# kaixi287/rsl_rl

Measured on AMD Instinct MI355X. Metric: PPO env-steps/sec (rollout+GAE+update) at N=65536 envs, 1→8 MI355X, higher is better.
Workload: dtype fp32

## Files before the change

rsl_rl_amd/csrc/mlp_fwd_stream.hip:

```cpp
#include <cstring>

#include "common.h"
#include "fwd_stream.h"
#include "mlp_tile.h"
#include "ppo_loss_common.h"
#include "x6_split.h"

namespace rslrl {
namespace {

constexpr int kFsT = 128;
constexpr int kFsN = 256;
constexpr int kFsThreads = 512;
constexpr int kFsChunkB = kFsT * 32;
constexpr int kFsMaxSlices = 128;
constexpr int kFsImgPlaneU = kX6PlaneB / 16;
constexpr int kFsImgChunkU = kX6ChunkB / 16;
static_assert(kFsT == kBM && kFsN == kBN && kFsThreads == kThreads, "the tiled kernel's tile (mlp_tile.h)");
constexpr uint32_t kFsRsrcFlags = 0x00020000;
#ifndef RSLRL_FS_LA
#define RSLRL_FS_LA 1
#endif
constexpr bool kFsLA = RSLRL_FS_LA != 0;

template <int K>
struct FsCfg {
    static constexpr int kChunks = K / 16;
    static constexpr int kStages = K == 256 ? 4 : 1;
    static constexpr int kNch = kChunks / kStages;
    static constexpr int kCols = 16 * kNch;
    static constexpr int kPlaneB = kNch * kFsChunkB;
    static constexpr int kBufB = 3 * kPlaneB;
    static constexpr int kUnitsRow = kCols / 4;
    static constexpr int kUpt = kFsT * kUnitsRow / kFsThreads;
    static_assert(K == 256 || K == 48, "streaming forward: K = 256 or 48");
    static_assert(kNch >= 2 && kUpt <= 4 && kFsT * kUnitsRow % kFsThreads == 0, "stage shape");
};

struct FsProblem {
    const float* x;
    const uint4* img;
    const float* bias;
    float* h;
};

struct FsArgs {
    FsProblem p[2];
    int tiles;
    int tiles_per;
};

__host__ __device__ constexpr int fs_f(int c) { return (c & 3) | ((c & 1) << 2); }

__device__ __forceinline__ int fs_off(int m, int col) {
    const int c = col >> 4;
    return c * kFsChunkB + (m ^ fs_f(c)) * 32 + 16 * (((col >> 3) & 1) ^ ((m >> 3) & 1)) + 8 * ((col >> 2) & 1);
}

__device__ __forceinline__ bf16x8 fs_read16(int addr) {
    typedef __attribute__((address_space(3))) uint4 lds_u4;
    return __builtin_bit_cast(bf16x8, *reinterpret_cast<const lds_u4*>(addr));
}

template <int K>
__device__ __forceinline__ void fs_load_x(__amdgpu_buffer_rsrc_t r, int q, float4 (&v)[4]) {
    using C = FsCfg<K>;
#pragma unroll
    for (int j = 0; j < C::kUpt; ++j) {
        const int u = threadIdx.x + kFsThreads * j;
        const int off = ((u / C::kUnitsRow) * K + 4 * (u % C::kUnitsRow)) * 4;
        v[j] = __builtin_bit_cast(float4, __builtin_amdgcn_raw_buffer_load_b128(r, off, q * C::kCols * 4, 2));
    }
}

template <int K>
__device__ __forceinline__ void fs_store_x1(const float4& v, int j, char* __restrict__ buf) {
    using C = FsCfg<K>;
    uint2 w[3];
    split4(v, w[0], w[1], w[2]);
    const int u = threadIdx.x + kFsThreads * j;
    const int off = fs_off(u / C::kUnitsRow, 4 * (u % C::kUnitsRow));
#pragma unroll
    for (int q = 0; q < 3; ++q) *reinterpret_cast<uint2*>(buf + q * C::kPlaneB + off) = w[q];
}

template <int K>
__global__ __launch_bounds__(kFsThreads, 1) void fwd_stream_kernel(FsArgs args) {
    using C = FsCfg<K>;
    __shared__ __attribute__((aligned(16))) char lds[2 * C::kBufB];
    const FsProblem& P = args.p[blockIdx.y];
    const int t_begin = blockIdx.x * args.tiles_per;
    const int t_end = min(args.tiles, t_begin + args.tiles_per);
    if (t_begin >= t_end) return;

    const int lane = threadIdx.x & 63;
    const int wave = __builtin_amdgcn_readfirstlane(threadIdx.x >> 6);
    if (wave >= 4) __builtin_amdgcn_s_setprio(1);
    const int h = lane >> 5;
    const int l32 = lane & 31;

    const int lbase = static_cast<int>(reinterpret_cast<uintptr_t>(lds));
    int la[2][C::kNch];
#pragma unroll
    for (int c = 0; c < C::kNch; ++c) {
        la[0][c] = lbase + fs_off(l32, 16 * c + 8 * h);
        la[1][c] = la[0][c] + C::kBufB;
    }
    const int brow = 32 * wave + l32;
    const int boff = (brow * 2 + (h ^ ((brow >> 3) & 1))) * 16;
    const __amdgpu_buffer_rsrc_t rimg = __builtin_amdgcn_make_buffer_rsrc(
        const_cast<uint4*>(P.img), 0, static_cast<uint32_t>(C::kChunks * kFsImgChunkU * 16), kFsRsrcFlags);
    auto bload = [&](int c, int q) {
        return __builtin_bit_cast(uint4, __builtin_amdgcn_raw_buffer_load_b128(rimg, boff, (c * kFsImgChunkU + q * kFsImgPlaneU) * 16, 0));
    };
    const float bias = P.bias[32 * wave + l32];

    auto tile_rsrc = [&](int tile) {
        return __builtin_amdgcn_make_buffer_rsrc(const_cast<float*>(P.x + static_cast<int64_t>(tile) * kFsT * K), 0,
                                                 static_cast<uint32_t>(kFsT * K * 4), kFsRsrcFlags);
    };

    float4 xr[4];
    fs_load_x<K>(tile_rsrc(t_begin), 0, xr);
#pragma unroll
    for (int j = 0; j < C::kUpt; ++j) fs_store_x1<K>(xr[j], j, lds);
    if (C::kStages > 1) fs_load_x<K>(tile_rsrc(t_begin), 1, xr);
    else if (t_begin + 1 < t_end) fs_load_x<K>(tile_rsrc(t_begin + 1), 0, xr);
    __syncthreads();

    uint4 bq[2][3];
#pragma unroll
    for (int q = 0; q < 3; ++q) bq[0][q] = bload(0, q);

    auto epi_part = [&](const f32x16 (&acc)[4], int tile, int e) {
        const __amdgpu_buffer_rsrc_t rc = __builtin_amdgcn_make_buffer_rsrc(
            P.h + static_cast<int64_t>(tile) * kFsT * kFsN + 32 * wave, 0, static_cast<uint32_t>(kFsT * kFsN * 4),
            kFsRsrcFlags);
        const int i = e >> 2;
#pragma unroll
        for (int k = 0; k < 4; ++k) {
            const int r = 4 * (e & 3) + k;
            float v = acc[i][r] + bias;
            const float n = elu_neg(fminf(v, 0.f));
            v = v > 0.f ? v : n;
            __builtin_amdgcn_raw_buffer_store_b32(__builtin_bit_cast(uint32_t, v), rc, ((4 * h + (r & 3)) * kFsN + l32) * 4,
                                                  (32 * i + 8 * (r >> 2)) * kFsN * 4, 2 );
        }
    };

    auto run_tile = [&](int tile, f32x16 (&acc)[4], const f32x16 (&prev)[4], bool has_prev, int par) {
        const bool more = tile + 1 < t_end;
#pragma unroll
        for (int kq = 0; kq < C::kStages; ++kq) {
            const int buf = (C::kStages % 2 == 0) ? (kq & 1) : (par ^ (kq & 1));
            bf16x8 an[3];
            if constexpr (kFsLA) {
                an[0] = fs_read16(la[buf][0]);
                an[1] = fs_read16(la[buf][0] + C::kPlaneB);
                an[2] = fs_read16(la[buf][0] + 2 * C::kPlaneB);
            }
            const bool next_stage = kq + 1 < C::kStages || more;
#pragma unroll
            for (int c = 0; c < C::kNch; ++c) {
                const int gc = C::kNch * kq + c;
                const int slot = (par * C::kChunks + gc) & 1;
#pragma unroll
                for (int q = 0; q < 3; ++q) bq[slot ^ 1][q] = bload((gc + 1) % C::kChunks, q);
                bf16x8 bf[3];
#pragma unroll
                for (int q = 0; q < 3; ++q) bf[q] = __builtin_bit_cast(bf16x8, bq[slot][q]);
#pragma unroll
                for (int i = 0; i < 4; ++i) {
                    const int blk = 4 * c + i;
                    bf16x8 af[3];
                    if constexpr (kFsLA) {
#pragma unroll
                        for (int q = 0; q < 3; ++q) af[q] = an[q];
                        if (blk + 1 < 4 * C::kNch) {
                            const int a1 = la[buf][(blk + 1) >> 2] + ((blk + 1) & 3) * 1024;
                            an[0] = fs_read16(a1);
                            an[1] = fs_read16(a1 + C::kPlaneB);
                            an[2] = fs_read16(a1 + 2 * C::kPlaneB);
                        }
                    } else {
                        const int a0 = la[buf][c] + i * 1024;
                        af[0] = fs_read16(a0);
                        af[1] = fs_read16(a0 + C::kPlaneB);
                        af[2] = fs_read16(a0 + 2 * C::kPlaneB);
                    }
                    acc[i] = mfma_x6(af, bf, gc == 0 ? f32x16{} : acc[i]);
                    if (kq == 0 && has_prev) {
                        if (blk < 16) epi_part(prev, tile - 1, blk);
                        if (blk == 4 * C::kNch - 1) {
#pragma unroll
                            for (int e = 4 * C::kNch; e < 16; ++e) epi_part(prev, tile - 1, e);
                        }
                    }
                    if (c == 1 && i < C::kUpt && next_stage) fs_store_x1<K>(xr[i], i, lds + (buf ^ 1) * C::kBufB);
                    __builtin_amdgcn_sched_barrier(0);
                }
                if (c == C::kNch - 1) {
                    if (C::kStages > 1) {
                        if (kq < C::kStages - 2 || more) {
                            const int s2 = kq + 2;
                            fs_load_x<K>(tile_rsrc(s2 < C::kStages ? tile : tile + 1), s2 % C::kStages, xr);
                        }
                    } else if (tile + 2 < t_end) {
                        fs_load_x<K>(tile_rsrc(tile + 2), 0, xr);
                    }
                    __builtin_amdgcn_sched_barrier(0);
                }
            }
            __syncthreads();
        }
    };

    f32x16 acc0[4], acc1[4];
    int tile = t_begin;
    for (; tile + 1 < t_end; tile += 2) {
        run_tile(tile, acc0, acc1, tile > t_begin, 0);
        run_tile(tile + 1, acc1, acc0, true, 1);
    }
    if (tile < t_end) {
        run_tile(tile, acc0, acc1, tile > t_begin, 0);
#pragma unroll
        for (int e = 0; e < 16; ++e) epi_part(acc0, tile, e);
    } else {
#pragma unroll
        for (int e = 0; e < 16; ++e) epi_part(acc1, tile - 1, e);
    }
}


struct VhArgs {
    const float* x;
    const uint4* img;
    const float* bias;
    const float* wv;
    float bv;
    const float* bvp;
    const float* tv;
    const float* ret;
    float* dz;
    float* y;
    float* wpart;
    float clip, g;
    int clipped;
    int tiles, tiles_per;
};
constexpr int kVhP = 260;

__global__ __launch_bounds__(kFsThreads, 1) void value_head_stream_kernel(VhArgs a) {
    using C = FsCfg<256>;
    __shared__ __attribute__((aligned(16))) char lds[2 * C::kBufB];
    __shared__ float red[8 * kFsT];
    __shared__ float dvl[kFsT];
    __shared__ float dbred[kFsT / 64];
    const int t_begin = blockIdx.x * a.tiles_per;
    const int t_end = min(a.tiles, t_begin + a.tiles_per);
    if (t_begin >= t_end) return;

    const int lane = threadIdx.x & 63;
    const int wave = __builtin_amdgcn_readfirstlane(threadIdx.x >> 6);
    if (wave >= 4) __builtin_amdgcn_s_setprio(1);
    const int h = lane >> 5;
    const int l32 = lane & 31;

    const int lbase = static_cast<int>(reinterpret_cast<uintptr_t>(lds));
    int la[2][C::kNch];
#pragma unroll
    for (int c = 0; c < C::kNch; ++c) {
        la[0][c] = lbase + fs_off(l32, 16 * c + 8 * h);
        la[1][c] = la[0][c] + C::kBufB;
    }
    const int brow = 32 * wave + l32;
    const int boff = (brow * 2 + (h ^ ((brow >> 3) & 1))) * 16;
    const __amdgpu_buffer_rsrc_t rimg = __builtin_amdgcn_make_buffer_rsrc(
        const_cast<uint4*>(a.img), 0, static_cast<uint32_t>(C::kChunks * kFsImgChunkU * 16), kFsRsrcFlags);
    auto bload = [&](int c, int q) {
        return __builtin_bit_cast(uint4, __builtin_amdgcn_raw_buffer_load_b128(rimg, boff, (c * kFsImgChunkU + q * kFsImgPlaneU) * 16, 0));
    };
    float bcol[16], wcol[16];
#pragma unroll
    for (int g = 0; g < 4; ++g) {
        const float4 b4 = *reinterpret_cast<const float4*>(a.bias + 32 * wave + 8 * g + 4 * h);
        const float4 w4 = *reinterpret_cast<const float4*>(a.wv + 32 * wave + 8 * g + 4 * h);
        bcol[4 * g] = b4.x; bcol[4 * g + 1] = b4.y; bcol[4 * g + 2] = b4.z; bcol[4 * g + 3] = b4.w;
        wcol[4 * g] = w4.x; wcol[4 * g + 1] = w4.y; wcol[4 * g + 2] = w4.z; wcol[4 * g + 3] = w4.w;
    }
    const float bv = *a.bvp;
    auto tile_rsrc = [&](int tile) {
        return __builtin_amdgcn_make_buffer_rsrc(const_cast<float*>(a.x + static_cast<int64_t>(tile) * kFsT * 256), 0,
                                                 static_cast<uint32_t>(kFsT * 256 * 4), kFsRsrcFlags);
    };

    float4 xr[4];
    fs_load_x<256>(tile_rsrc(t_begin), 0, xr);
#pragma unroll
    for (int j = 0; j < C::kUpt; ++j) fs_store_x1<256>(xr[j], j, lds);
    fs_load_x<256>(tile_rsrc(t_begin), 1, xr);
    __syncthreads();

    uint4 bq[2][3];
#pragma unroll
    for (int q = 0; q < 3; ++q) bq[0][q] = bload(0, q);

    float wacc[16];
#pragma unroll
    for (int r = 0; r < 16; ++r) wacc[r] = 0.f;
    float dbacc = 0.f;

    for (int tile = t_begin; tile < t_end; ++tile) {
        const bool more = tile + 1 < t_end;
        const int64_t row0 = static_cast<int64_t>(tile) * kFsT;
        f32x16 acc[4];
#pragma unroll
        for (int kq = 0; kq < 4; ++kq) {
            const int buf = kq & 1;
            bf16x8 an[3];
            an[0] = fs_read16(la[buf][0]);
            an[1] = fs_read16(la[buf][0] + C::kPlaneB);
            an[2] = fs_read16(la[buf][0] + 2 * C::kPlaneB);
#pragma unroll
            for (int c = 0; c < C::kNch; ++c) {
                const int gc = C::kNch * kq + c;
                const int slot = gc & 1;
#pragma unroll
                for (int q = 0; q < 3; ++q) bq[slot ^ 1][q] = bload((gc + 1) % C::kChunks, q);
                bf16x8 bf[3];
#pragma unroll
                for (int q = 0; q < 3; ++q) bf[q] = __builtin_bit_cast(bf16x8, bq[slot][q]);
#pragma unroll
                for (int i = 0; i < 4; ++i) {
                    const int blk = 4 * c + i;
                    bf16x8 af[3];
#pragma unroll
                    for (int q = 0; q < 3; ++q) af[q] = an[q];
                    if (blk + 1 < 4 * C::kNch) {
                        const int a1 = la[buf][(blk + 1) >> 2] + ((blk + 1) & 3) * 1024;
                        an[0] = fs_read16(a1);
                        an[1] = fs_read16(a1 + C::kPlaneB);
                        an[2] = fs_read16(a1 + 2 * C::kPlaneB);
                    }
                    acc[i] = mfma_x6(bf, af, gc == 0 ? f32x16{} : acc[i]);
                    if (c == 1 && i < C::kUpt && (kq < 3 || more)) fs_store_x1<256>(xr[i], i, lds + (buf ^ 1) * C::kBufB);
                    __builtin_amdgcn_sched_barrier(0);
                }
                if (c == C::kNch - 1) {
                    if (kq < 2 || more) fs_load_x<256>(tile_rsrc(kq < 2 ? tile : tile + 1), (kq + 2) & 3, xr);
                    __builtin_amdgcn_sched_barrier(0);
                }
            }
            __syncthreads();
        }
        float tvr = 0.f, retr = 0.f;
        if (threadIdx.x < kFsT) {
            tvr = a.tv[row0 + threadIdx.x];
            retr = a.ret[row0 + threadIdx.x];
        }
#pragma unroll
        for (int i = 0; i < 4; ++i) {
            float oval = 0.f;
#pragma unroll
            for (int r = 0; r < 16; ++r) {
                const float tt = acc[i][r] + bcol[r];
                const float n = elu_neg(fminf(tt, 0.f));
                const float hv = tt > 0.f ? tt : n;
                acc[i][r] = hv;
                oval = fmaf(hv, wcol[r], oval);
            }
            const float tsum = oval + __shfl_xor(oval, 32, 64);
            if (h == 0) red[wave * kFsT + 32 * i + l32] = tsum;
        }
        __syncthreads();
        if (threadIdx.x < kFsT) {
            const int rl = threadIdx.x;
            float V = red[rl];
#pragma unroll
            for (int w = 1; w < 8; ++w) V += red[w * kFsT + rl];
            V += bv;
            a.y[row0 + rl] = V;
            const float dV = value_loss_grad(V, tvr, retr, a.clipped, a.clip, a.g);
            dvl[rl] = dV;
            dbacc += dV;
        }
        __syncthreads();
        float* dzt = a.dz + row0 * 256 + 32 * wave + 4 * h;
#pragma unroll
        for (int i = 0; i < 4; ++i) {
            const float dv = dvl[32 * i + l32];
#pragma unroll
            for (int g = 0; g < 4; ++g) {
                float o[4];
#pragma unroll
                for (int k = 0; k < 4; ++k) {
                    const int r = 4 * g + k;
                    const float hh = acc[i][r];
                    const float z = __fmaf_rn(dv, wcol[r], 0.f);
                    o[k] = hh > 0.f ? z : z * (hh + 1.f);
                    wacc[r] = fmaf(dv, hh, wacc[r]);
                }
                const f32x4 ov = {o[0], o[1], o[2], o[3]};
                *reinterpret_cast<f32x4*>(dzt + (32 * i + l32) * 256 + 8 * g) = ov;
            }
        }
    }
    float* wp = a.wpart + static_cast<int64_t>(blockIdx.x) * kVhP;
#pragma unroll
    for (int r = 0; r < 16; ++r) {
        float v = wacc[r];
#pragma unroll
        for (int off = 1; off < 32; off <<= 1) v += __shfl_xor(v, off, 64);
        wacc[r] = v;
    }
    if (l32 == 0) {
#pragma unroll
        for (int g = 0; g < 4; ++g)
            *reinterpret_cast<float4*>(wp + 32 * wave + 8 * g + 4 * h) =
                make_float4(wacc[4 * g], wacc[4 * g + 1], wacc[4 * g + 2], wacc[4 * g + 3]);
    }
    if (threadIdx.x < kFsT) {
        float v = dbacc;
#pragma unroll
        for (int off = 1; off < 64; off <<= 1) v += __shfl_xor(v, off, 64);
        if (lane == 0) dbred[wave] = v;
    }
    __syncthreads();
    if (threadIdx.x == 0) {
        wp[256] = dbred[0] + dbred[1];
        wp[257] = 0.f;
        wp[258] = 0.f;
        wp[259] = 0.f;
    }
}

int64_t fs_tiles_per(int64_t tiles) { return ceil_div(tiles, std::min<int64_t>(kFsMaxSlices, tiles)); }

}

bool fwd_stream_forced() {
    static const bool on = [] {
        const char* e = std::getenv("RSLRL_FWD_STREAM");
        return e && (std::strcmp(e, "1") == 0 || std::strcmp(e, "48") == 0);
    }();
    return on;
}

bool fwd_stream48() {
    static const bool on = [] {
        const char* e = std::getenv("RSLRL_FWD_STREAM");
        return e && std::strcmp(e, "48") == 0;
    }();
    return on;
}

bool fwd_stream_enabled() {
    static const bool on = [] {
        const char* e = std::getenv("RSLRL_FWD_STREAM");
        return !(e && e[0] == '0');
    }();
    return on;
}

int fwd_stream_pair(const FwdStreamProblem* p, int n, int64_t M, int K, hipStream_t st) {
    if (n < 1 || n > 2 || M <= 0 || M % kFsT || M / kFsT > INT32_MAX || (K != 256 && K != 48))
        return RSLRL_E_UNSUPPORTED;
    FsArgs args{};
    for (int i = 0; i < n; ++i) {
        const uintptr_t bits = reinterpret_cast<uintptr_t>(p[i].x) | reinterpret_cast<uintptr_t>(p[i].img);
        if (!p[i].x || !p[i].img || !p[i].bias || !p[i].h) return RSLRL_E_INVALID_ARGUMENT;
        if (bits & 15) return RSLRL_E_MISALIGNED;
        args.p[i] = FsProblem{p[i].x, static_cast<const uint4*>(p[i].img), p[i].bias, p[i].h};
    }
    const int64_t tiles = M / kFsT;
    const int64_t per = fs_tiles_per(tiles);
    args.tiles = static_cast<int>(tiles);
    args.tiles_per = static_cast<int>(per);
    const dim3 grid(static_cast<unsigned>(ceil_div(tiles, per)), static_cast<unsigned>(n));
    if (K == 256) hipLaunchKernelGGL(fwd_stream_kernel<256>, grid, dim3(kFsThreads), 0, st, args);
    else hipLaunchKernelGGL(fwd_stream_kernel<48>, grid, dim3(kFsThreads), 0, st, args);
    return launch_status();
}


int value_head_stream(const ValueHeadStreamArgs& v, hipStream_t st) {
    if (v.M <= 0 || v.M % kFsT || v.M / kFsT > INT32_MAX) return RSLRL_E_UNSUPPORTED;
    const uintptr_t bits = reinterpret_cast<uintptr_t>(v.x) | reinterpret_cast<uintptr_t>(v.img) |
                           reinterpret_cast<uintptr_t>(v.bias) | reinterpret_cast<uintptr_t>(v.wv) |
                           reinterpret_cast<uintptr_t>(v.dz) | reinterpret_cast<uintptr_t>(v.wpart);
    if (bits & 15) return RSLRL_E_MISALIGNED;
    const int64_t tiles = v.M / kFsT;
    const int64_t per = ceil_div(tiles, std::min<int64_t>(2 * kFsMaxSlices, tiles));
    VhArgs a{};
    a.x = v.x;
    a.img = static_cast<const uint4*>(v.img);
    a.bias = v.bias;
    a.wv = v.wv;
    a.bvp = v.bv;
    a.tv = v.tv;
    a.ret = v.ret;
    a.dz = v.dz;
    a.y = v.y;
    a.wpart = v.wpart;
    a.clip = v.clip;
    a.g = v.g;
    a.clipped = v.clipped;
    a.tiles = static_cast<int>(tiles);
    a.tiles_per = static_cast<int>(per);
    hipLaunchKernelGGL(value_head_stream_kernel, dim3(static_cast<unsigned>(ceil_div(tiles, per))), dim3(kFsThreads), 0,
                       st, a);
    return launch_status();
}

int64_t value_head_stream_rows(int64_t M) {
    if (M <= 0 || M % kFsT) return 0;
    const int64_t tiles = M / kFsT;
    const int64_t per = ceil_div(tiles, std::min<int64_t>(2 * kFsMaxSlices, tiles));
    return ceil_div(tiles, per);
}

bool value_head_stream_enabled() {
    static const bool on = [] {
        const char* e = std::getenv("RSLRL_VALUE_HEAD_STREAM");
        return !(e && e[0] == '0');
    }();
    return on;
}
}
```

Measured before the change: 18.87 million.

## Overlap value-head epilogue of previous tile with next tile's MFMA main loop

Result: no change. 18.94 million, median of 6 (+0.4%).

```diff
diff --git a/rsl_rl_amd/csrc/mlp_fwd_stream.hip b/rsl_rl_amd/csrc/mlp_fwd_stream.hip
--- a/rsl_rl_amd/csrc/mlp_fwd_stream.hip
+++ b/rsl_rl_amd/csrc/mlp_fwd_stream.hip
@@ -249,13 +249,17 @@
     int tiles, tiles_per;
 };
 constexpr int kVhP = 260;
-
+constexpr bool kVhOverlapDefault = true;
+
+template <bool kOverlap>
 __global__ __launch_bounds__(kFsThreads, 1) void value_head_stream_kernel(VhArgs a) {
     using C = FsCfg<256>;
     __shared__ __attribute__((aligned(16))) char lds[2 * C::kBufB];
     __shared__ float red[8 * kFsT];
     __shared__ float dvl[kFsT];
     __shared__ float dbred[kFsT / 64];
+    __shared__ __attribute__((aligned(16))) float btab[kOverlap ? kFsN : 4];
+    __shared__ __attribute__((aligned(16))) float wtab[kOverlap ? kFsN : 4];
     const int t_begin = blockIdx.x * a.tiles_per;
     const int t_end = min(a.tiles, t_begin + a.tiles_per);
     if (t_begin >= t_end) return;
@@ -281,24 +285,57 @@
         return __builtin_bit_cast(uint4, __builtin_amdgcn_raw_buffer_load_b128(rimg, boff, (c * kFsImgChunkU + q * kFsImgPlaneU) * 16, 0));
     };
     float bcol[16], wcol[16];
-#pragma unroll
-    for (int g = 0; g < 4; ++g) {
-        const float4 b4 = *reinterpret_cast<const float4*>(a.bias + 32 * wave + 8 * g + 4 * h);
-        const float4 w4 = *reinterpret_cast<const float4*>(a.wv + 32 * wave + 8 * g + 4 * h);
-        bcol[4 * g] = b4.x; bcol[4 * g + 1] = b4.y; bcol[4 * g + 2] = b4.z; bcol[4 * g + 3] = b4.w;
-        wcol[4 * g] = w4.x; wcol[4 * g + 1] = w4.y; wcol[4 * g + 2] = w4.z; wcol[4 * g + 3] = w4.w;
-    }
+    if constexpr (kOverlap) {
+        if (threadIdx.x < kFsN) {
+            btab[threadIdx.x] = a.bias[threadIdx.x];
+            wtab[threadIdx.x] = a.wv[threadIdx.x];
+        }
+    } else {
+#pragma unroll
+        for (int g = 0; g < 4; ++g) {
+            const float4 b4 = *reinterpret_cast<const float4*>(a.bias + 32 * wave + 8 * g + 4 * h);
+            const float4 w4 = *reinterpret_cast<const float4*>(a.wv + 32 * wave + 8 * g + 4 * h);
+            bcol[4 * g] = b4.x; bcol[4 * g + 1] = b4.y; bcol[4 * g + 2] = b4.z; bcol[4 * g + 3] = b4.w;
+            wcol[4 * g] = w4.x; wcol[4 * g + 1] = w4.y; wcol[4 * g + 2] = w4.z; wcol[4 * g + 3] = w4.w;
+        }
+    }
+    auto col4 = [&](const float (&reg)[16], const float* tab, int g, float (&o)[4]) {
+        if constexpr (kOverlap) {
+            int off = 4 * h;
+            asm volatile("" : "+v"(off));
+            const float4 v = *reinterpret_cast<const float4*>(tab + 32 * wave + 8 * g + off);
+            o[0] = v.x; o[1] = v.y; o[2] = v.z; o[3] = v.w;
+        } else {
+#pragma unroll
+            for (int k = 0; k < 4; ++k) o[k] = reg[4 * g + k];
+        }
+    };
     const float bv = *a.bvp;
     auto tile_rsrc = [&](int tile) {
         return __builtin_amdgcn_make_buffer_rsrc(const_cast<float*>(a.x + static_cast<int64_t>(tile) * kFsT * 256), 0,
                                                  static_cast<uint32_t>(kFsT * 256 * 4), kFsRsrcFlags);
     };
 
+    const int xg = ((threadIdx.x / C::kUnitsRow) * 256 + 4 * (threadIdx.x % C::kUnitsRow)) * 4;
+    const int xl = fs_off(threadIdx.x / C::kUnitsRow, 4 * (threadIdx.x % C::kUnitsRow));
+    static_assert(kFsThreads / C::kUnitsRow == 32 && C::kUpt == 4, "unit j = unit 0 + 32 j rows");
     float4 xr[4];
-    fs_load_x<256>(tile_rsrc(t_begin), 0, xr);
-#pragma unroll
-    for (int j = 0; j < C::kUpt; ++j) fs_store_x1<256>(xr[j], j, lds);
-    fs_load_x<256>(tile_rsrc(t_begin), 1, xr);
+    auto load_x = [&](__amdgpu_buffer_rsrc_t r, int q) {
+#pragma unroll
+        for (int j = 0; j < 4; ++j)
+            xr[j] = __builtin_bit_cast(float4, __builtin_amdgcn_raw_buffer_load_b128(r, xg, q * C::kCols * 4 + j * 32 * 256 * 4, 2));
+    };
+    auto store_x1 = [&](int j, int buf) {
+        uint2 w[3];
+        split4(xr[j], w[0], w[1], w[2]);
+#pragma unroll
+        for (int q = 0; q < 3; ++q)
+            *reinterpret_cast<uint2*>(lds + xl + (buf * C::kBufB + q * C::kPlaneB + j * 1024)) = w[q];
+    };
+    load_x(tile_rsrc(t_begin), 0);
+#pragma unroll
+    for (int j = 0; j < 4; ++j) store_x1(j, 0);
+    load_x(tile_rsrc(t_begin), 1);
     __syncthreads();
 
     uint4 bq[2][3];
@@ -309,18 +346,103 @@
 #pragma unroll
     for (int r = 0; r < 16; ++r) wacc[r] = 0.f;
     float dbacc = 0.f;
-
-    for (int tile = t_begin; tile < t_end; ++tile) {
+    float tvr = 0.f, retr = 0.f;
+    float oval = 0.f;
+    float dvc = 0.f;
+
+    auto row_rsrc = [&](const float* p, int tile) {
+        return __builtin_amdgcn_make_buffer_rsrc(const_cast<float*>(p + static_cast<int64_t>(tile) * kFsT), 0,
+                                                 static_cast<uint32_t>(kFsT * 4), kFsRsrcFlags);
+    };
+    auto load_targets = [&](int tile) {
+        if (wave < kFsT / 64) {
+            tvr = __builtin_bit_cast(float, __builtin_amdgcn_raw_buffer_load_b32(row_rsrc(a.tv, tile), 4 * threadIdx.x, 0, 0));
+            retr = __builtin_bit_cast(float, __builtin_amdgcn_raw_buffer_load_b32(row_rsrc(a.ret, tile), 4 * threadIdx.x, 0, 0));
+        }
+    };
+    auto stage_a = [&](f32x16 (&acc)[4], int i, int g) {
+        float b4[4], w4[4];
+        col4(bcol, btab, g, b4);
+        col4(wcol, wtab, g, w4);
+        if (g == 0) oval = 0.f;
+#pragma unroll
+        for (int k = 0; k < 4; ++k) {
+            const int r = 4 * g + k;
+            const float tt = acc[i][r] + b4[k];
+            const float n = elu_neg(fminf(tt, 0.f));
+            const float hv = tt > 0.f ? tt : n;
+            acc[i][r] = hv;
+            oval = fmaf(hv, w4[k], oval);
+        }
+        if (g == 3) {
+            const float tsum = oval + __shfl_xor(oval, 32, 64);
+            if (h == 0) red[wave * kFsT + 32 * i + l32] = tsum;
+        }
+    };
+    auto stage_b = [&](int tile) {
+        if (wave < kFsT / 64) {
+            const int rl = threadIdx.x;
+            float V = red[rl];
+#pragma unroll
+            for (int w = 1; w < 8; ++w) V += red[w * kFsT + rl];
+            V += bv;
+            __builtin_amdgcn_raw_buffer_store_b32(__builtin_bit_cast(uint32_t, V), row_rsrc(a.y, tile), 4 * rl, 0, 0);
+            const float dV = value_loss_grad(V, tvr, retr, a.clipped, a.clip, a.g);
+            dvl[rl] = dV;
+            dbacc += dV;
+        }
+    };
+    auto stage_c = [&](const f32x16 (&acc)[4], int tile, int i, int g) {
+        const uint64_t dzb = reinterpret_cast<uint64_t>(a.dz + static_cast<int64_t>(tile) * kFsT * 256 + 32 * wave + 32 * i * 256 + 8 * g);
+        const uint32_t dzlo = __builtin_amdgcn_readfirstlane(static_cast<uint32_t>(dzb));
+        const uint32_t dzhi = __builtin_amdgcn_readfirstlane(static_cast<uint32_t>(dzb >> 32));
+        typedef __attribute__((address_space(1))) f32x4 global_f32x4;
+        if (g == 0) dvc = dvl[32 * i + l32];
+        float w4[4];
+        col4(wcol, wtab, g, w4);
+        float o[4];
+#pragma unroll
+        for (int k = 0; k < 4; ++k) {
+            const int r = 4 * g + k;
+            const float hh = acc[i][r];
+            const float z = __fmaf_rn(dvc, w4[k], 0.f);
+            o[k] = hh > 0.f ? z : z * (hh + 1.f);
+            wacc[r] = fmaf(dvc, hh, wacc[r]);
+        }
+        const f32x4 ov = {o[0], o[1], o[2], o[3]};
+        *reinterpret_cast<global_f32x4*>((static_cast<uint64_t>(dzhi) << 32 | dzlo) +
+                                         static_cast<uint32_t>((l32 * 256 + 4 * h) * 4)) = ov;
+    };
+    auto drain = [&](f32x16 (&acc)[4], int tile) {
+        load_targets(tile);
+#pragma unroll
+        for (int i = 0; i < 4; ++i) {
+#pragma unroll
+            for (int g = 0; g < 4; ++g) stage_a(acc, i, g);
+        }
+        __syncthreads();
+        stage_b(tile);
+        __syncthreads();
+#pragma unroll
+        for (int i = 0; i < 4; ++i) {
+#pragma unroll
+            for (int g = 0; g < 4; ++g) stage_c(acc, tile, i, g);
+        }
+    };
+
+    auto run_tile = [&](int tile, f32x16 (&acc)[4], f32x16 (&prev)[4], bool has_prev) {
         const bool more = tile + 1 < t_end;
-        const int64_t row0 = static_cast<int64_t>(tile) * kFsT;
-        f32x16 acc[4];
+        const bool epi = kOverlap && has_prev;
 #pragma unroll
         for (int kq = 0; kq < 4; ++kq) {
             const int buf = kq & 1;
+            const bool look = !(kOverlap && kq == 0);
             bf16x8 an[3];
-            an[0] = fs_read16(la[buf][0]);
-            an[1] = fs_read16(la[buf][0] + C::kPlaneB);
-            an[2] = fs_read16(la[buf][0] + 2 * C::kPlaneB);
+            if (look) {
+                an[0] = fs_read16(la[buf][0]);
+                an[1] = fs_read16(la[buf][0] + C::kPlaneB);
+                an[2] = fs_read16(la[buf][0] + 2 * C::kPlaneB);
+            }
 #pragma unroll
             for (int c = 0; c < C::kNch; ++c) {
                 const int gc = C::kNch * kq + c;
@@ -334,75 +456,62 @@
                 for (int i = 0; i < 4; ++i) {
                     const int blk = 4 * c + i;
                     bf16x8 af[3];
-#pragma unroll
-                    for (int q = 0; q < 3; ++q) af[q] = an[q];
-                    if (blk + 1 < 4 * C::kNch) {
-                        const int a1 = la[buf][(blk + 1) >> 2] + ((blk + 1) & 3) * 1024;
-                        an[0] = fs_read16(a1);
-                        an[1] = fs_read16(a1 + C::kPlaneB);
-                        an[2] = fs_read16(a1 + 2 * C::kPlaneB);
+                    if (look) {
+#pragma unroll
+                        for (int q = 0; q < 3; ++q) af[q] = an[q];
+                        if (blk + 1 < 4 * C::kNch) {
+                            const int a1 = la[buf][(blk + 1) >> 2] + ((blk + 1) & 3) * 1024;
+                            an[0] = fs_read16(a1);
+                            an[1] = fs_read16(a1 + C::kPlaneB);
+                            an[2] = fs_read16(a1 + 2 * C::kPlaneB);
+                        }
+                    } else {
+                        const int a0 = la[buf][c] + i * 1024;
+                        af[0] = fs_read16(a0);
+                        af[1] = fs_read16(a0 + C::kPlaneB);
+                        af[2] = fs_read16(a0 + 2 * C::kPlaneB);
                     }
                     acc[i] = mfma_x6(bf, af, gc == 0 ? f32x16{} : acc[i]);
-                    if (c == 1 && i < C::kUpt && (kq < 3 || more)) fs_store_x1<256>(xr[i], i, lds + (buf ^ 1) * C::kBufB);
+                    if constexpr (kOverlap) {
+                        if (epi) {
+                            if (kq == 0) stage_a(prev, blk >> 2, blk & 3);
+                            if (kq == 1 && blk == 0) stage_b(tile - 1);
+                            if (kq == 2) stage_c(prev, tile - 1, blk >> 2, blk & 3);
+                        }
+                    }
+                    if (c == 1 && (kq < 3 || more)) store_x1(i, buf ^ 1);
                     __builtin_amdgcn_sched_barrier(0);
                 }
                 if (c == C::kNch - 1) {
-                    if (kq < 2 || more) fs_load_x<256>(tile_rsrc(kq < 2 ? tile : tile + 1), (kq + 2) & 3, xr);
+                    if (kq < 2 || more) load_x(tile_rsrc(kq < 2 ? tile : tile + 1), (kq + 2) & 3);
+                    if constexpr (kOverlap) {
+                        if (kq == 0 && epi) load_targets(tile - 1);
+                    }
                     __builtin_amdgcn_sched_barrier(0);
                 }
             }
             __syncthreads();
         }
-        float tvr = 0.f, retr = 0.f;
-        if (threadIdx.x < kFsT) {
-            tvr = a.tv[row0 + threadIdx.x];
-            retr = a.ret[row0 + threadIdx.x];
-        }
-#pragma unroll
-        for (int i = 0; i < 4; ++i) {
-            float oval = 0.f;
-#pragma unroll
-            for (int r = 0; r < 16; ++r) {
-                const float tt = acc[i][r] + bcol[r];
-                const float n = elu_neg(fminf(tt, 0.f));
-                const float hv = tt > 0.f ? tt : n;
-                acc[i][r] = hv;
-                oval = fmaf(hv, wcol[r], oval);
-            }
-            const float tsum = oval + __shfl_xor(oval, 32, 64);
-            if (h == 0) red[wave * kFsT + 32 * i + l32] = tsum;
-        }
-        __syncthreads();
-        if (threadIdx.x < kFsT) {
-            const int rl = threadIdx.x;
-            float V = red[rl];
-#pragma unroll
-            for (int w = 1; w < 8; ++w) V += red[w * kFsT + rl];
-            V += bv;
-            a.y[row0 + rl] = V;
-            const float dV = value_loss_grad(V, tvr, retr, a.clipped, a.clip, a.g);
-            dvl[rl] = dV;
-            dbacc += dV;
-        }
-        __syncthreads();
-        float* dzt = a.dz + row0 * 256 + 32 * wave + 4 * h;
-#pragma unroll
-        for (int i = 0; i < 4; ++i) {
-            const float dv = dvl[32 * i + l32];
-#pragma unroll
-            for (int g = 0; g < 4; ++g) {
-                float o[4];
-#pragma unroll
-                for (int k = 0; k < 4; ++k) {
-                    const int r = 4 * g + k;
-                    const float hh = acc[i][r];
-                    const float z = __fmaf_rn(dv, wcol[r], 0.f);
-                    o[k] = hh > 0.f ? z : z * (hh + 1.f);
-                    wacc[r] = fmaf(dv, hh, wacc[r]);
-                }
-                const f32x4 ov = {o[0], o[1], o[2], o[3]};
-                *reinterpret_cast<f32x4*>(dzt + (32 * i + l32) * 256 + 8 * g) = ov;
-            }
+    };
+
+    f32x16 acc0[4];
+    if constexpr (kOverlap) {
+        f32x16 acc1[4];
+        int tile = t_begin;
+        for (; tile + 1 < t_end; tile += 2) {
+            run_tile(tile, acc0, acc1, tile > t_begin);
+            run_tile(tile + 1, acc1, acc0, true);
+        }
+        if (tile < t_end) {
+            run_tile(tile, acc0, acc1, tile > t_begin);
+            drain(acc0, tile);
+        } else {
+            drain(acc1, tile - 1);
+        }
+    } else {
+        for (int tile = t_begin; tile < t_end; ++tile) {
+            run_tile(tile, acc0, acc0, false);
+            drain(acc0, tile);
         }
     }
     float* wp = a.wpart + static_cast<int64_t>(blockIdx.x) * kVhP;
@@ -507,8 +616,11 @@
     a.clipped = v.clipped;
     a.tiles = static_cast<int>(tiles);
     a.tiles_per = static_cast<int>(per);
-    hipLaunchKernelGGL(value_head_stream_kernel, dim3(static_cast<unsigned>(ceil_div(tiles, per))), dim3(kFsThreads), 0,
-                       st, a);
+    const char* e = std::getenv("RSLRL_VALUE_HEAD_EPI");
+    const bool overlap = e && e[0] ? std::strcmp(e, "serial") != 0 : kVhOverlapDefault;
+    const dim3 grid(static_cast<unsigned>(ceil_div(tiles, per)));
+    if (overlap) hipLaunchKernelGGL(value_head_stream_kernel<true>, grid, dim3(kFsThreads), 0, st, a);
+    else hipLaunchKernelGGL(value_head_stream_kernel<false>, grid, dim3(kFsThreads), 0, st, a);
     return launch_status();
 }
 
```
